# Kerollmops/oxidized-mtbl

Measured on AMD Instinct MI355X. Metric: KV records/s + GiB/s of block bytes decoded, device-resident, higher is better.
Workload: dtype u8; 1 GPU; cfg2: 4 KiB blocks, 16 B keys / 64 B values, restart_interval=16, compression=none, device-resident decode; blocks_per_gpu=100000, block_bytes_per_gpu=401800126, records_per_gpu=5100000, key_bytes_per_gpu=81600000, parallelism=block-sharded x1, no collective

## Files before the change

oxidized-mtbl_amd/csrc/decode.hip:

```cpp
#include <hip/hip_runtime.h>
#include <stdint.h>

#include <stdlib.h>

#include <algorithm>

#include "bounds.h"
#include "devinfo.h"
#include "crc_dev.h"
#include "mtblx.h"

#if (defined(MTBLX_ABL_NOKEY) || defined(MTBLX_ABL_NOVAL) || defined(MTBLX_ABL_NOVSTORE) || \
     defined(MTBLX_ABL_CRC) || defined(MTBLX_SPILL)) && !defined(MTBLX_DIAG)
#error "ablation / spill knobs are diagnostic: build them through a Makefile diagnostic target (-DMTBLX_DIAG)"
#endif

namespace mtblx {

constexpr int kWave = 64;
constexpr uint64_t kU32Max = 0xFFFFFFFFull;
constexpr uint32_t kNotStaged = 0xFFFFFFFFu;
constexpr uint32_t kOutOfBounds = 0xFFFFFFFEu;

__device__ __forceinline__ uint32_t byte_of(const uint4& w, uint32_t t) {
// ... 214 lines not shown
  static constexpr int MAXINT = MAXINT_;
  static constexpr int MAXBLK = MAXBLK_;
  static constexpr bool VALPOS = false;
};

struct Rec {
  uint32_t pos_sh;
  uint32_t ns_vl;
  uint32_t ks;
  uint32_t vs_blk;
};

template <class C>
struct alignas(16) TileLds {
  uint8_t stage[C::TB];
  Rec rec[C::MAXREC];
  uint32_t boff[C::MAXBLK];
  uint32_t blen[C::MAXBLK];
  uint32_t bR[C::MAXBLK];
  uint32_t bn[C::MAXBLK];
  uint32_t bint0[C::MAXBLK + 1];
  uint32_t bok[C::MAXBLK];
  uint32_t bwr[C::MAXBLK];
  int32_t bst[C::MAXBLK];
  uint32_t bcnt[C::MAXBLK], bkb[C::MAXBLK], bvb[C::MAXBLK];
  uint32_t brb[C::MAXBLK], bkbb[C::MAXBLK], bvbb[C::MAXBLK];
  uint32_t brf[C::MAXBLK];
  uint32_t icnt[C::MAXINT + 1], ikb[C::MAXINT + 1], ivb[C::MAXINT + 1];
  uint8_t iblk[C::MAXINT];
  uint64_t tpre[3];
  uint64_t tinc[3];
  uint32_t ttot[3];
  uint32_t nfastrec;
  uint32_t contig;
  uint32_t wsum[4][3];
  uint64_t lbsum[4][3];
};

struct TileArgs {
  const uint8_t* data;
  uint64_t data_len;
  const uint64_t* blk_off;
  const uint32_t* blk_len;
  uint32_t nblk;
  uint32_t bpt;
  uint32_t slot;
  uint32_t ntiles;
  uint32_t* nrec;
  uint64_t* rec_base;
  uint64_t* key_base;
  uint64_t* val_base;
  int32_t* status;
  uint32_t* key_end;
  uint32_t* val_end;
  uint64_t rec_cap;
  uint8_t* keys;
  uint64_t keys_cap;
  uint8_t* vals;
  uint64_t vals_cap;
  uint64_t* totals;
  uint64_t* lbw;
  struct WsHdr* hdr;
  uint64_t* dbg;
  int write;
  uint32_t* crc;
  uint8_t* crc_bad;
  int crc_framed;
  uint32_t wscap;
  uint32_t par;
  uint32_t hw_other;
  unsigned long long inject;
  uint32_t flags_direct;
  uint64_t wait_ticks;
  uint64_t dbg_delay0;
  uint32_t* val_pos;
};

struct WsHdr {
  uint32_t epoch;
  uint32_t done;
  uint32_t hw[2];
  unsigned long long flags;
  unsigned long long tflags[2];
};

__device__ __forceinline__ void tile_span(const TileArgs& a, uint32_t t, uint32_t& b0, uint32_t& nb) {
  b0 = t * a.bpt;
  nb = min(a.bpt, a.nblk - b0);
}

constexpr int kTileWords = 4;
__device__ __forceinline__ uint64_t* lb_slot(const TileArgs& a, uint64_t t) { return a.lbw + kTileWords * t + a.par; }
__device__ __forceinline__ uint64_t* lbx_slot(const TileArgs& a, uint64_t t) { return a.lbw + kTileWords * t + 2; }
__device__ __forceinline__ uint64_t* lbx2_slot(const TileArgs& a, uint64_t t) { return a.lbw + kTileWords * t + 3; }

__device__ __forceinline__ bool fits_at(uint64_t base, uint64_t n, uint64_t cap) { return base <= cap && n <= cap - base; }

__device__ __forceinline__ void ws_begin(TileArgs& a) {
  const uint32_t ep = __hip_atomic_load(&a.hdr->epoch, __ATOMIC_RELAXED, __HIP_MEMORY_SCOPE_AGENT);
  a.par = ep & 1u;
  a.hw_other = __hip_atomic_load(&a.hdr->hw[a.par ^ 1u], __ATOMIC_RELAXED, __HIP_MEMORY_SCOPE_AGENT);
  if (a.hw_other > a.wscap) a.hw_other = a.wscap;
  const uint32_t n = blockDim.x, tid = threadIdx.x;
  for (uint64_t t = (uint64_t)blockIdx.x * n + tid; t < a.hw_other; t += (uint64_t)gridDim.x * n)
    a.lbw[kTileWords * t + (a.par ^ 1u)] = 0;
  if (blockIdx.x == 0 && tid == 0)
    __hip_atomic_store(&a.hdr->tflags[a.par ^ 1u], 0ull, __ATOMIC_RELAXED, __HIP_MEMORY_SCOPE_AGENT);
}

__device__ __forceinline__ void ws_debug_delay(const TileArgs& a) {
  if (blockIdx.x == 0 && a.dbg_delay0) {
    const uint64_t t0 = __builtin_amdgcn_s_memrealtime();
    while (__builtin_amdgcn_s_memrealtime() - t0 < a.dbg_delay0) __builtin_amdgcn_s_sleep(127);
  }
}

__device__ __forceinline__ void ws_flag(const TileArgs& a, unsigned long long bit) {
  atomicOr(a.flags_direct ? reinterpret_cast<unsigned long long*>(a.totals + 3) : &a.hdr->flags, bit);
}

__device__ __forceinline__ void ws_timeout(const TileArgs& a) {
  if (a.flags_direct) {
    __hip_atomic_fetch_or(&a.hdr->tflags[a.par], 2ull, __ATOMIC_RELAXED, __HIP_MEMORY_SCOPE_AGENT);
    asm volatile("s_waitcnt vmcnt(0)" ::: "memory");
  }
  ws_flag(a, 2ull);
}

constexpr uint64_t kWaitTicks = 20ull * 100000000ull;
struct WaitBound {
  uint64_t t0 = 0;
  uint32_t n = 0;
  __device__ __forceinline__ bool expired(uint64_t ticks) {
    if ((++n & 63u) != 0u) return false;
    const uint64_t t = __builtin_amdgcn_s_memrealtime();
    if (t0 == 0) t0 = t;
    return t - t0 > ticks;
  }
};

__device__ __forceinline__ void ws_end(const TileArgs& a) {
  __syncthreads();
  if (threadIdx.x == 0) {
    const uint32_t old = __hip_atomic_fetch_add(&a.hdr->done, 1u, __ATOMIC_RELAXED, __HIP_MEMORY_SCOPE_AGENT);
    if (old == gridDim.x - 1) {
      const unsigned long long f = __hip_atomic_exchange(&a.hdr->flags, 0ull, __ATOMIC_RELAXED, __HIP_MEMORY_SCOPE_AGENT);
      a.totals[3] = f | a.inject;
      __hip_atomic_fetch_max(&a.hdr->hw[a.par], a.ntiles, __ATOMIC_RELAXED, __HIP_MEMORY_SCOPE_AGENT);
      __hip_atomic_exchange(&a.hdr->done, 0u, __ATOMIC_RELAXED, __HIP_MEMORY_SCOPE_AGENT);
      __hip_atomic_fetch_add(&a.hdr->epoch, 1u, __ATOMIC_RELAXED, __HIP_MEMORY_SCOPE_AGENT);
    }
  }
}


__device__ __forceinline__ void pipe_zero_flags(const TileArgs& a) {
  unsigned long long* tot = reinterpret_cast<unsigned long long*>(a.totals + 3);
  __hip_atomic_store(tot, 0ull, __ATOMIC_RELAXED, __HIP_MEMORY_SCOPE_AGENT);
  asm volatile("s_waitcnt vmcnt(0)" ::: "memory");
  const unsigned long long early = __hip_atomic_load(&a.hdr->tflags[a.par], __ATOMIC_RELAXED, __HIP_MEMORY_SCOPE_AGENT);
  if (early) __hip_atomic_fetch_or(tot, early, __ATOMIC_RELAXED, __HIP_MEMORY_SCOPE_AGENT);
  asm volatile("s_waitcnt vmcnt(0)" ::: "memory");
}

__device__ __forceinline__ void pipe_close(const TileArgs& a) {
  if (a.inject) __hip_atomic_fetch_or(a.totals + 3, a.inject, __ATOMIC_RELAXED, __HIP_MEMORY_SCOPE_AGENT);
  __hip_atomic_fetch_max(&a.hdr->hw[a.par], a.ntiles, __ATOMIC_RELAXED, __HIP_MEMORY_SCOPE_AGENT);
  __hip_atomic_fetch_add(&a.hdr->epoch, 1u, __ATOMIC_RELAXED, __HIP_MEMORY_SCOPE_AGENT);
}

__device__ __forceinline__ void tile_range(const TileArgs& a, uint32_t t, uint32_t tb, uint64_t& r0, uint64_t& r1) {
  uint32_t b0, nb;
  tile_span(a, t, b0, nb);
  MTBLX_CHK(a.blk_off + b0, 8 * nb);
  MTBLX_CHK(a.blk_len + b0, 4 * nb);
  const uint64_t s = a.blk_off[b0];
  const uint64_t e = a.blk_off[b0 + nb - 1] + a.blk_len[b0 + nb - 1];
  const uint64_t base = reinterpret_cast<uintptr_t>(a.data);
  r0 = ((base + s) & ~15ull) - base;
  if (base + s < 16 || ((base + s) & ~15ull) < base) r0 = 0;
  r1 = (e > s && e - r0 + 48 <= tb) ? e : 0;
  for (uint32_t j = 1; r1 && j + 1 < nb; ++j)
    if (a.blk_off[b0 + j] < s || a.blk_off[b0 + j] + a.blk_len[b0 + j] > e) r1 = 0;
}

__device__ __forceinline__ uint4 load_chunk(const TileArgs& a, uint64_t off) {
  if (off + 16 <= a.data_len) {
    MTBLX_CHK(a.data + off, 16);
    return *reinterpret_cast<const uint4*>(a.data + off);
  }
  uint32_t t[4] = {0, 0, 0, 0};
  for (int i = 0; i < 16; ++i)
    if (off + i < a.data_len) MTBLX_CHK(a.data + off + i, 1), t[i >> 2] |= (uint32_t)a.data[off + i] << (8 * (i & 3));
  return make_uint4(t[0], t[1], t[2], t[3]);
}

__device__ __forceinline__ uint32_t stage_slot(const TileArgs& a, uint8_t* slot, uint64_t off, uint32_t L, int lane) {
  const uint64_t base = reinterpret_cast<uintptr_t>(a.data);
  const uint64_t a0 = ((base + off) & ~15ull) - base;
  const uint32_t delta = (uint32_t)(off - a0);
  const uint32_t nch = (delta + L + 15u) >> 4;
  for (uint32_t c = lane; c < nch; c += kWave) *reinterpret_cast<uint4*>(slot + 16 * c) = load_chunk(a, a0 + 16ull * c);
  return delta;
}

template <bool WRITE>
__device__ __forceinline__ bool walk_interval(const uint8_t* stage, Rec* recs, uint32_t bo, uint32_t L, uint32_t R, uint32_t s,
                                              uint32_t e, uint32_t& cnt, uint32_t& kb, uint32_t& vb, uint32_t slot0,
                                              uint32_t kbase, uint32_t vbase, uint32_t blk, uint32_t rlo,
                                              uint32_t rhi) {
  cnt = kb = vb = 0;
  if (!(s < e && e <= R)) return false;
  uint32_t p = s, prevlen = 0;
  const uint32_t* st32 = reinterpret_cast<const uint32_t*>(stage);
  while (p < e) {
    const uint32_t ad = bo + p;
    uint32_t hw = (MTBLX_LCHK(st32 + (ad >> 2), 8), __builtin_amdgcn_alignbit(st32[(ad >> 2) + 1], st32[ad >> 2], (ad & 3u) * 8u));
    uint32_t sh = hw & 0xffu, ns = (hw >> 8) & 0xffu, vl = (hw >> 16) & 0xffu, h = 3;
    if (__builtin_expect((hw & 0x808080u) != 0u, 0)) {
      if (R - p < 3u) return false;
      uint4 W = lds_win16(stage, ad);
      uint32_t l0 = dec32(W, 0, L - p, sh);
      if (l0 == 0) return false;
      uint32_t l1 = dec32(W, l0, L - p - l0, ns);
      if (l1 == 0) return false;
      uint32_t l2 = dec32(W, l0 + l1, L - p - l0 - l1, vl);
      if (l2 == 0) return false;
      h = l0 + l1 + l2;
      if (p + h > R) return false;
      if ((sh | ns | vl) > 0xFFFFu) return false;
    }
    if (R - p < h + ns + vl) return false;
    if (sh > prevlen) return false;
    const uint32_t klen = sh + ns;
    if (WRITE) {
      const uint32_t r = slot0 + cnt;
      if (r >= rlo && r < rhi) {
// ... 419 lines not shown
              --sidx;
              const uint32_t x = S.rec[sidx].pos_sh;
              shs = x >> 16;
              ps = x & 0xFFFFu;
            }
            const uint32_t seg = m < jend ? m : jend;
            const uint32_t src = bo + ps + (jj - shs);
            uint4 w4 = lds_win16(S.stage, src - (jj - j0));
            merge_bytes(outw, w4, (int)(jj - j0), (int)(seg - j0));
            jj = seg;
          }
          store_bytes(kd + j0, outw, jend - j0);
        }
#endif
      }
      __syncthreads();
      if (fb >= nint) break;
      plan_chunk(fb);
      walk2();
      __syncthreads();
    }
    STAMP(6);

    if (tid < (int)nb && !S.bok[tid] && S.bwr[tid]) {
      const uint32_t j = tid, bo = S.boff[j], L = S.blen[j];
      const uint8_t* d = (bo != kNotStaged) ? (S.stage + bo) : (a.data + a.blk_off[b0 + j]);
      if constexpr (C::VALPOS)
        generic_block<true, true>(d, L, a.keys + pk + S.bkbb[j], nullptr, a.key_end + pr + S.brb[j],
                                  a.val_end + pr + S.brb[j], a.val_pos + pr + S.brb[j]);
      else
        generic_block<true>(d, L, a.keys + pk + S.bkbb[j], a.vals + pv + S.bvbb[j], a.key_end + pr + S.brb[j],
                            a.val_end + pr + S.brb[j]);
    }
    __syncthreads();
  }
  ws_end(a);
#ifdef MTBLX_STAMPS
  if (tid == 0 && a.dbg) {
    for (int k = 0; k < 8; ++k) atomicAdd(reinterpret_cast<unsigned long long*>(a.dbg + k), (unsigned long long)tacc[k]);
    atomicAdd(reinterpret_cast<unsigned long long*>(a.dbg + 8), (unsigned long long)ntl);
  }
#endif
}

struct Stamps {
#ifdef MTBLX_STAMPS
  uint64_t acc[15] = {0, 0, 0, 0, 0, 0, 0, 0, 0, 0, 0, 0, 0, 0, 0};
  uint64_t prev = 0;
  __device__ __forceinline__ void init() { prev = __builtin_amdgcn_s_memtime(); }
  __device__ __forceinline__ void hit(int k) {
    const uint64_t t = __builtin_amdgcn_s_memtime();
    acc[k] += t - prev;
    prev = t;
  }
#else
  __device__ __forceinline__ void init() {}
  __device__ __forceinline__ void hit(int) {}
#endif
};

#ifdef MTBLX_STAMPS
__device__ uint64_t g_tl[1024][16];
#define TL(k) do { if (threadIdx.x == 0 && blockIdx.x < 1024) g_tl[blockIdx.x][k] = __builtin_amdgcn_s_memrealtime(); } while (0)
#define TLW(k) do { if ((threadIdx.x & 63) == 0 && blockIdx.x < 1024) g_tl[blockIdx.x][k] = __builtin_amdgcn_s_memrealtime(); } while (0)
#else
#define TL(k) do { } while (0)
#define TLW(k) do { } while (0)
#endif

constexpr int kPipeThreads = 1024;
constexpr int kPipeLoadWave = 2;
constexpr int kP2Spi = 16;
constexpr uint32_t kLargeDmaSplit = 24;

template <int TB_, int NBUF_, int MAXBLK_, int MAXINT_, bool VERIFY_ = false, int LOADW_ = 2>
struct PipeCfg {
  static constexpr int TB = TB_, NBUF = NBUF_, MAXBLK = MAXBLK_, MAXINT = MAXINT_;
  static constexpr int SLOTS = MAXINT * kP2Spi;
  static constexpr bool VERIFY = VERIFY_;
  static constexpr int LOADW = LOADW_;
  static constexpr int COPY0 = kPipeLoadWave + LOADW;
  static constexpr int NCOPY = kPipeThreads / kWave - COPY0;
  static constexpr int ROWS = NCOPY * (kWave / 16);
  static constexpr bool VALPOS = false;
};
#ifndef MTBLX_SMALL_TB
#define MTBLX_SMALL_TB 49664
#endif
using PipeSmall = PipeCfg<MTBLX_SMALL_TB, 3, 16, 56>;
#ifndef MTBLX_LARGE_LOADW
#define MTBLX_LARGE_LOADW 2
#endif
using PipeLarge = PipeCfg<65664, 2, 2, 64, false, MTBLX_LARGE_LOADW>;
using PipeSmallV = PipeCfg<49152, 3, 16, 56, true>;
using PipeLargeV = PipeCfg<65664, 2, 2, 64, true>;
struct PipeSmallP : PipeSmall { static constexpr bool VALPOS = true; };
struct PipeLargeP : PipeLarge { static constexpr bool VALPOS = true; };

template <class P>
struct alignas(16) PipeBuf {
  uint8_t stage[P::TB];
  uint16_t pos[P::SLOTS];
  uint32_t boff[P::MAXBLK], blen[P::MAXBLK];
  uint32_t bok[P::MAXBLK], bwr[P::MAXBLK];
  int32_t bst[P::MAXBLK];
  uint32_t bcnt[P::MAXBLK], bkb[P::MAXBLK], bvb[P::MAXBLK];
  uint32_t brb[P::MAXBLK], bkbb[P::MAXBLK], bvbb[P::MAXBLK];
  uint32_t icnt[P::MAXINT + 1], ikb[P::MAXINT + 1], ivb[P::MAXINT + 1];
  uint8_t iraw[P::MAXINT];
  uint8_t iblk[P::MAXINT];
  uint64_t tpre[3];
  uint32_t ttot[3];
  uint32_t nb, b0, nint;
};

template <class P>
struct alignas(16) PipeLds {
  PipeBuf<P> buf[P::NBUF];
  uint32_t ready;
  uint32_t pub;
  uint32_t cdone;
  uint32_t staged;
  uint8_t cmk[kPipeThreads / kWave][kWave];
  uint32_t crcT[P::VERIFY ? 4 : 1][P::VERIFY ? 256 : 1];
  uint32_t cacc[2][P::VERIFY ? P::MAXBLK : 1];
  uint32_t cst[2][P::VERIFY ? P::MAXBLK : 1];
  uint32_t cfr[2][P::VERIFY ? P::MAXBLK : 1];
  uint32_t shK[P::VERIFY ? 64 : 1];
  uint32_t shX[P::VERIFY ? 32 : 1];
  uint32_t crcdone;
};

__device__ __forceinline__ void raw_barrier() {
  asm volatile("s_waitcnt lgkmcnt(0)\n\ts_barrier" ::: "memory");
}

template <int D>
__device__ __forceinline__ uint32_t row_shr_keep(uint32_t x) {
  return (uint32_t)__builtin_amdgcn_update_dpp((int)x, (int)x, 0x110 + D, 0xf, 0xf, false);
}
template <int D>
__device__ __forceinline__ uint32_t row_shr_zero(uint32_t x) {
  return (uint32_t)__builtin_amdgcn_update_dpp(0, (int)x, 0x110 + D, 0xf, 0xf, false);
}

__device__ __forceinline__ uint32_t row_excl_scan(uint32_t x) {
  uint32_t y = x;
  y += row_shr_zero<1>(y);
  y += row_shr_zero<2>(y);
  y += row_shr_zero<4>(y);
  y += row_shr_zero<8>(y);
  return y - x;
}

__device__ __forceinline__ uint32_t keep_mask(int t, int i) {
  int lo = t - 4 * i;
  lo = lo < 0 ? 0 : lo;
  return lo >= 4 ? 0u : (0xFFFFFFFFu << (8 * lo));
}

template <int D>
__device__ __forceinline__ void key_scan_step(uint32_t& m, uint4& W, uint32_t q0) {
  const uint32_t mL = row_shr_keep<D>(m);
  uint4 L;
  L.x = row_shr_keep<D>(W.x);
  L.y = row_shr_keep<D>(W.y);
// ... 113 lines not shown
    kb += klen;
    vb += vl;
    prevlen = klen;
    p += h + ns + vl;
  }
  return p == e && (prevlen <= 0xFFFFu);
}

template <class P>
__device__ __forceinline__ void pipe_dma(PipeBuf<P>& B, const TileArgs& a, uint32_t t, uint64_t off_l, uint32_t len_l,
                                         int lane, uint32_t part, uint32_t mlo = 0, uint32_t mhi = 0xFFFFFFFFu) {
  typedef __attribute__((address_space(3))) void lds_void;
  typedef __attribute__((address_space(1))) const void g_void;
  uint32_t b0, nb;
  tile_span(a, t, b0, nb);
  const uint64_t base = reinterpret_cast<uintptr_t>(a.data);
  const uint64_t s = ((uint64_t)(uint32_t)__builtin_amdgcn_readlane((int)(off_l >> 32), 0) << 32) |
                     (uint32_t)__builtin_amdgcn_readlane((int)(uint32_t)off_l, 0);
  const uint64_t end_l = off_l + len_l;
  const uint64_t e = ((uint64_t)(uint32_t)__builtin_amdgcn_readlane((int)(end_l >> 32), (int)nb - 1) << 32) |
                     (uint32_t)__builtin_amdgcn_readlane((int)(uint32_t)end_l, (int)nb - 1);
  uint64_t r0 = ((base + s) & ~15ull) - base;
  if (base + s < 16 || ((base + s) & ~15ull) < base) r0 = 0;
  const bool inside = off_l >= s && end_l <= e;
  const bool contig = e > s && e - r0 + 48 <= (uint64_t)P::TB && __ballot(!inside) == 0ull;
  if (contig) {
    const uint32_t nch = (uint32_t)((e - r0 + 15) >> 4);
    const bool al = ((base + r0) & 15ull) == 0;
    const uint64_t room = a.data_len > r0 ? (a.data_len - r0) / 16u : 0u;
    const uint32_t nfull = al ? (uint32_t)min<uint64_t>(nch, room) : 0u;
    const uint32_t mfull = min(nfull / kWave, mhi);
    uint32_t m = part + ((mlo + P::LOADW - 1 - part) / P::LOADW) * P::LOADW;
    if (mlo <= part) m = part;
    const uint8_t* gp = a.data + r0 + 16ull * ((uint64_t)m * kWave + (uint32_t)lane);
    for (; m < mfull; m += P::LOADW, gp += 16 * kWave * P::LOADW)
      MTBLX_CHK(gp, 16), MTBLX_LCHK(B.stage + 16 + 1024 * m, 1024), __builtin_amdgcn_global_load_lds((g_void*)gp, (lds_void*)(B.stage + 16 + 1024 * m), 16, 0, MTBLX_DMA_AUX);
    for (; m * kWave < nch && m < mhi; m += P::LOADW) {
      const uint32_t c = m * kWave + lane;
      const uint64_t go = r0 + 16ull * c;
      if (c < nfull)
        MTBLX_CHK(a.data + go, 16), MTBLX_LCHK(B.stage + 16 + 1024 * m, 1024), __builtin_amdgcn_global_load_lds((g_void*)(a.data + go), (lds_void*)(B.stage + 16 + 1024 * m), 16, 0, MTBLX_DMA_AUX);
      else if (c < nch)
        *reinterpret_cast<uint4*>(B.stage + 16 + 16 * c) = load_chunk(a, go);
    }
    if (part == 0 && lane < (int)nb) {
      B.boff[lane] = off_l + len_l > a.data_len ? kOutOfBounds : (uint32_t)(16 + off_l - r0);
      B.blen[lane] = len_l;
    }
  } else if (mlo == 0) {
    for (uint32_t j = 0; j < nb; ++j) {
      const uint64_t off = ((uint64_t)(uint32_t)__builtin_amdgcn_readlane((int)(off_l >> 32), (int)j) << 32) |
                           (uint32_t)__builtin_amdgcn_readlane((int)(uint32_t)off_l, (int)j);
      const uint32_t L = (uint32_t)__builtin_amdgcn_readlane((int)len_l, (int)j);
      const uint32_t so = 16u + j * a.slot;
      uint32_t bo = kNotStaged;
      if (off + L > a.data_len) {
        bo = kOutOfBounds;
      } else if (L + 15u <= a.slot && so + a.slot + 32u <= (uint32_t)P::TB) {
        uint64_t a0 = ((base + off) & ~15ull) - base;
        if (base + off < 16 || ((base + off) & ~15ull) < base) a0 = off;
        const uint32_t delta = (uint32_t)(off - a0);
        const uint32_t nch = (delta + L + 15u) >> 4;
        for (uint32_t m = part; m * kWave < nch; m += P::LOADW) {
          const uint32_t c = m * kWave + lane;
          const uint64_t go = a0 + 16ull * c;
          if (c < nch) {
            if (go + 16 <= a.data_len && ((base + go) & 15ull) == 0)
              MTBLX_CHK(a.data + go, 16), MTBLX_LCHK(B.stage + so + 1024 * m, 1024), __builtin_amdgcn_global_load_lds((g_void*)(a.data + go), (lds_void*)(B.stage + so + 1024 * m), 16, 0,
                                               MTBLX_DMA_AUX);
            else
              *reinterpret_cast<uint4*>(B.stage + so + 16 * c) = load_chunk(a, go);
          }
        }
        bo = so + delta;
      }
      if (part == 0 && lane == 0) { B.boff[j] = bo; B.blen[j] = L; }
    }
  }
  if (part == 0 && lane == 0) { B.nb = nb; B.b0 = b0; }
}

template <class P>
__device__ __forceinline__ void pipe_walk(PipeBuf<P>& B, const TileArgs& a, uint32_t t, int lane, Stamps& ST,
                                          uint32_t& wmode) {
  uint32_t b0, nb;
  tile_span(a, t, b0, nb);
  uint32_t n = 0, R = 0, ok = 0, L = 0, bo = kNotStaged;
  if (lane < (int)nb) {
    L = B.blen[lane];
    bo = B.boff[lane];
    if (bo < kOutOfBounds && L >= 8) {
      n = lds_rd32(B.stage, bo + L - 4);
      if (n != 0 && (uint64_t)(n + 1ull) * 4ull <= L) { R = L - 4u * (n + 1u); ok = 1; }
    }
  }
  uint32_t incl = wave_incl_scan(ok ? n : 0u);
  if (ok && incl > (uint32_t)P::MAXINT) ok = 0;
  n = ok ? n : 0;
  incl = wave_incl_scan(n);
  const uint32_t bint0 = incl - n;
  const uint32_t nint = (uint32_t)__builtin_amdgcn_readlane((int)incl, (int)nb - 1);
  uint32_t j = 0;
  for (uint32_t b = 0; b + 1 < nb; ++b) j += ((uint32_t)__builtin_amdgcn_readlane((int)incl, (int)b) <= (uint32_t)lane);
  const int js = (int)j;
  const uint32_t jbo = (uint32_t)__shfl((int)bo, js, kWave), jR = (uint32_t)__shfl((int)R, js, kWave);
  const uint32_t jn = (uint32_t)__shfl((int)n, js, kWave), jb0 = (uint32_t)__shfl((int)bint0, js, kWave);
  const uint32_t jL = (uint32_t)__shfl((int)L, js, kWave);
  ST.hit(9);
  const bool fl = (uint32_t)lane < nint;
  uint32_t cnt = 0, kb = 0, vb = 0;
  bool wok = false, need2 = false;
  if (fl) {
    const uint32_t i = (uint32_t)lane - jb0;
    const uint32_t s = lds_rd32(B.stage, jbo + jR + 4u * i);
    const uint32_t e = (i + 1 < jn) ? lds_rd32(B.stage, jbo + jR + 4u * (i + 1)) : jR;
    ST.hit(10);
    const uint32_t slot0 = (uint32_t)lane * kP2Spi;
    bool all1 = true;
    constexpr bool kAdaptive = P::NBUF == 2 && !P::VERIFY;
    if (!kAdaptive || wmode == 0u) {
      wok = e <= jR && walk_pos(B.stage, B.pos, jbo, s, e, slot0, cnt, kb, vb);
      if (!wok) {
        wok = e <= jR && walk_pos2(B.stage, B.pos, jbo, s, e, slot0, cnt, kb, vb, all1);
        all1 = false;
      }
    } else {
      wok = e <= jR && walk_pos2(B.stage, B.pos, jbo, s, e, slot0, cnt, kb, vb, all1);
      all1 = all1 || !wok;
    }
    need2 = !all1;
    if (!wok) wok = walk_careful_pos(B.stage, B.pos, jbo, jL, jR, s, e, slot0, cnt, kb, vb);
    B.iraw[lane] = (uint8_t)(cnt < 255u ? cnt : 255u);
    B.iblk[lane] = (uint8_t)j;
  }
  ST.hit(2);
  if constexpr (P::NBUF == 2 && !P::VERIFY) wmode = __ballot(need2) != 0ull ? 1u : 0u;
  const uint64_t failm = __ballot(fl && !wok);
  {
    const uint64_t hi = incl >= 64u ? ~0ull : ((1ull << incl) - 1ull);
    const uint64_t lo = (1ull << bint0) - 1ull;
    if (ok && (failm & hi & ~lo) != 0ull) ok = 0;
  }
  const bool jok = __shfl((int)ok, js, kWave) != 0;
  uint32_t gc = 0, gk = 0, gv = 0;
  int32_t gst = MTBLX_ST_OK;
  if (lane < (int)nb && !ok) {
    if (bo == kNotStaged) MTBLX_CHK(a.blk_off + b0 + lane, 8);
    const uint8_t* d = (bo != kNotStaged) ? (B.stage + bo) : (a.data + a.blk_off[b0 + lane]);
    const GenOut o = bo == kOutOfBounds ? GenOut{0, 0, 0, MTBLX_ST_CORRUPT}
                                        : generic_block<false>(d, L, nullptr, nullptr, nullptr, nullptr);
    gc = o.nrec; gk = (uint32_t)o.kb; gv = (uint32_t)o.vb; gst = o.st;
  }
  const uint32_t gwr = ok || gen_writable(bo, gst);
  const bool reg = fl && jok;
  const uint32_t c = reg ? cnt : 0u, k = reg ? kb : 0u, v = reg ? vb : 0u;
  const uint32_t ic = wave_incl_scan(c), ik = wave_incl_scan(k), iv = wave_incl_scan(v);
  const uint32_t tr = (uint32_t)__builtin_amdgcn_readlane((int)ic, 63) + wave_sum32(gc);
  const uint32_t tk = (uint32_t)__builtin_amdgcn_readlane((int)ik, 63) + wave_sum32(gk);
  const uint32_t tv = (uint32_t)__builtin_amdgcn_readlane((int)iv, 63) + wave_sum32(gv);
  if (lane == 0) {
    if (t == 0) pipe_zero_flags(a);
    lb_publish(a, t, tr, tk, tv);
    B.ttot[0] = tr; B.ttot[1] = tk; B.ttot[2] = tv;
    B.nint = nint;
  }
  if (nb == 1) {
    const uint32_t n0 = (uint32_t)__builtin_amdgcn_readlane((int)incl, 0);
    const uint32_t tc = n0 ? (uint32_t)__builtin_amdgcn_readlane((int)ic, (int)n0 - 1) : 0u;
    const uint32_t tkk = n0 ? (uint32_t)__builtin_amdgcn_readlane((int)ik, (int)n0 - 1) : 0u;
    const uint32_t tvv = n0 ? (uint32_t)__builtin_amdgcn_readlane((int)iv, (int)n0 - 1) : 0u;
    if (lane == 0) {
      B.bok[0] = ok; B.bwr[0] = gwr; B.bst[0] = ok ? MTBLX_ST_OK : gst;
      B.bcnt[0] = ok ? tc : gc; B.bkb[0] = ok ? tkk : gk; B.bvb[0] = ok ? tvv : gv;
      B.brb[0] = 0; B.bkbb[0] = 0; B.bvbb[0] = 0;
    }
    if (fl) {
      B.icnt[lane] = ic - c;
      B.ikb[lane] = ik - k;
      B.ivb[lane] = iv - v;
    }
    return;
  }
  const int ea_l = bint0 ? (int)bint0 - 1 : 0, eb_l = incl ? (int)incl - 1 : 0;
  const uint32_t ea0 = (uint32_t)__shfl((int)ic, ea_l, kWave), eb0 = (uint32_t)__shfl((int)ic, eb_l, kWave);
  const uint32_t ka0 = (uint32_t)__shfl((int)ik, ea_l, kWave), kb0 = (uint32_t)__shfl((int)ik, eb_l, kWave);
  const uint32_t va0 = (uint32_t)__shfl((int)iv, ea_l, kWave), vb0 = (uint32_t)__shfl((int)iv, eb_l, kWave);
  uint32_t bc = 0, bk = 0, bv = 0;
  if (lane < (int)nb) {
    if (ok) {
      bc = (incl ? eb0 : 0u) - (bint0 ? ea0 : 0u);
      bk = (incl ? kb0 : 0u) - (bint0 ? ka0 : 0u);
      bv = (incl ? vb0 : 0u) - (bint0 ? va0 : 0u);
    } else {
      bc = gc; bk = gk; bv = gv;
    }
  }
  const uint32_t jc = wave_incl_scan(bc), jk = wave_incl_scan(bk), jv = wave_incl_scan(bv);
  const uint32_t brb = jc - bc, bkbb = jk - bk, bvbb = jv - bv;
  if (lane < (int)nb) {
    B.bok[lane] = ok; B.bwr[lane] = gwr; B.bst[lane] = ok ? MTBLX_ST_OK : gst;
    B.bcnt[lane] = bc; B.bkb[lane] = bk; B.bvb[lane] = bv;
    B.brb[lane] = brb; B.bkbb[lane] = bkbb; B.bvbb[lane] = bvbb;
  }
  const uint32_t jea = (uint32_t)__shfl((int)(bint0 ? ea0 : 0u), js, kWave);
  const uint32_t jka = (uint32_t)__shfl((int)(bint0 ? ka0 : 0u), js, kWave);
  const uint32_t jva = (uint32_t)__shfl((int)(bint0 ? va0 : 0u), js, kWave);
  const uint32_t jrb = (uint32_t)__shfl((int)brb, js, kWave), jkb = (uint32_t)__shfl((int)bkbb, js, kWave),
                 jvb = (uint32_t)__shfl((int)bvbb, js, kWave);
  if (fl) {
    B.icnt[lane] = jrb + (ic - c) - jea;
    B.ikb[lane] = jkb + (ik - k) - jka;
    B.ivb[lane] = jvb + (iv - v) - jva;
  }
}

__device__ __forceinline__ void pipe_lookback_issue(const TileArgs& a, uint32_t t, uint32_t G,
                                                    uint64_t lbv[kMaxLookbackLoads], int lane) {
  const int64_t lo = (t >= G) ? (int64_t)t - G + 1 : 0;
#pragma unroll
  for (int m = 0; m < kMaxLookbackLoads; ++m) {
    const int64_t i = (int64_t)t - 1 - lane - (int64_t)m * kWave;
    lbv[m] = (i >= lo) ? __hip_atomic_load(lb_slot(a, i), __ATOMIC_RELAXED, __HIP_MEMORY_SCOPE_AGENT) : kReady;
  }
}

__device__ __forceinline__ void pipe_lookback_poll(const TileArgs& a, uint32_t t, uint32_t G,
                                                   uint64_t lbv[kMaxLookbackLoads], int lane, const uint32_t* cdone,
                                                   uint32_t want) {
  const int64_t lo = (t >= G) ? (int64_t)t - G + 1 : 0;
  for (uint32_t spin = 0; spin < (1u << 22); ++spin) {
    bool pend = false;
#pragma unroll
    for (int m = 0; m < kMaxLookbackLoads; ++m) {
      const int64_t i = (int64_t)t - 1 - lane - (int64_t)m * kWave;
      pend |= (i >= lo) && !(lbv[m] & kReady);
    }
    if (__ballot(pend) == 0ull) return;
    if (__hip_atomic_load(cdone, __ATOMIC_RELAXED, __HIP_MEMORY_SCOPE_WORKGROUP) >= want) return;
    __builtin_amdgcn_s_sleep(2);
#pragma unroll
    for (int m = 0; m < kMaxLookbackLoads; ++m) {
      const int64_t i = (int64_t)t - 1 - lane - (int64_t)m * kWave;
      if (i >= lo && !(lbv[m] & kReady)) lbv[m] = __hip_atomic_load(lb_slot(a, i), __ATOMIC_RELAXED, __HIP_MEMORY_SCOPE_AGENT);
    }
  }
}

template <class P>
__device__ __forceinline__ void pipe_lookback(PipeBuf<P>& B, const TileArgs& a, uint32_t t, uint32_t G, uint64_t tinc[3],
                                              uint64_t lbv[kMaxLookbackLoads], int lane, uint32_t* ready,
                                              uint32_t rv) {
  const uint32_t nb = B.nb, b0 = B.b0;
  const int64_t lo = (t >= G) ? (int64_t)t - G + 1 : 0;
  uint64_t sr = 0, sk = 0, sv = 0;
  bool timeout = false;
#pragma unroll
  for (int m = 0; m < kMaxLookbackLoads; ++m) {
    const int64_t i = (int64_t)t - 1 - lane - (int64_t)m * kWave;
    uint64_t w = lbv[m];
    WaitBound wb;
    while (!(w & kReady)) {
      __builtin_amdgcn_s_sleep(2);
      w = __hip_atomic_load(lb_slot(a, i), __ATOMIC_RELAXED, __HIP_MEMORY_SCOPE_AGENT);
      if (wb.expired(a.wait_ticks)) { timeout = true; w = kReady; }
    }
    if (i < lo) continue;
    lb_take(a, (uint64_t)i, w, sr, sk, sv);
  }
  if (timeout) ws_timeout(a);
  sr = lb_wave_sum(sr);
  sv = lb_wave_sum(sv);
  sk = lb_wave_sum(sk);
  const uint64_t pr = tinc[0] + sr, pk = tinc[1] + sk, pv = tinc[2] + sv;
  tinc[0] = pr + B.ttot[0];
  tinc[1] = pk + B.ttot[1];
  tinc[2] = pv + B.ttot[2];
  if (lane == 0) {
    B.tpre[0] = pr; B.tpre[1] = pk; B.tpre[2] = pv;
    if (t == a.ntiles - 1) MTBLX_CHK(a.totals, 24);
    if (t == a.ntiles - 1) { a.totals[0] = tinc[0]; a.totals[1] = tinc[1]; a.totals[2] = tinc[2]; }
  }
  const bool fits = !a.write || (fits_at(pr, B.ttot[0], a.rec_cap) && fits_at(pk, B.ttot[1], a.keys_cap) &&
                                 fits_at(pv, B.ttot[2], a.vals_cap));
  if (fits) {
    __builtin_amdgcn_fence(__ATOMIC_RELEASE, "workgroup");
    if (lane == 0) __hip_atomic_store(ready, rv, __ATOMIC_RELEASE, __HIP_MEMORY_SCOPE_WORKGROUP);
  }
  if (lane < (int)nb) {
    const uint32_t j = lane, b = b0 + j;
    const uint64_t rb = pr + B.brb[j], kb = pk + B.bkbb[j], vb = pv + B.bvbb[j];
    MTBLX_CHK(a.nrec + b, 4);
    MTBLX_CHK(a.rec_base + b, 8);
    MTBLX_CHK(a.key_base + b, 8);
    MTBLX_CHK(a.val_base + b, 8);
    MTBLX_CHK(a.status + b, 4);
    a.nrec[b] = B.bcnt[j];
    a.rec_base[b] = rb;
    a.key_base[b] = kb;
    a.val_base[b] = vb;
    int32_t st = B.bst[j];
    if (a.write && !(fits_at(rb, B.bcnt[j], a.rec_cap) && fits_at(kb, B.bkb[j], a.keys_cap) &&
                     fits_at(vb, B.bvb[j], a.vals_cap))) {
      st = MTBLX_ST_OVERFLOW;
      B.bwr[j] = 0;
      ws_flag(a, 1ull);
    }
    a.status[b] = st;
  }
  if (!fits) {
    __builtin_amdgcn_fence(__ATOMIC_RELEASE, "workgroup");
    if (lane == 0) __hip_atomic_store(ready, rv, __ATOMIC_RELEASE, __HIP_MEMORY_SCOPE_WORKGROUP);
  }
}

struct CopyRow {
  uint32_t f, j, k, bo, sh, ns, vl, klen, ks, vs, sp, m0;
  uint4 W0;
  bool fv, live;
};

template <class P>
__device__ __forceinline__ CopyRow copy_prepare(const PipeBuf<P>& B, uint32_t fb, int lane) {
  CopyRow r;
  const uint32_t nint = B.nint;
  r.k = lane & 15;
  r.f = fb + (lane >> 4);
  r.fv = r.f < nint;
  r.j = r.fv ? B.iblk[r.f] : 0u;
  r.live = r.fv && r.k < B.iraw[r.f] && B.bok[r.j];
  r.bo = B.boff[r.j];
  const uint32_t p = r.live ? B.pos[r.f * kP2Spi + r.k] : 0u;
  uint32_t sh = 0, ns = 0, vl = 0, h = 3;
  if (r.live) {
    const uint32_t hw = lds_rd32(B.stage, r.bo + p);
    sh = hw & 0xffu; ns = (hw >> 8) & 0xffu; vl = (hw >> 16) & 0xffu;
    if ((hw & 0x808080u) != 0u) {
      const uint4 W = lds_win16(B.stage, r.bo + p);
      const uint32_t l0 = dec32(W, 0, 16, sh);
      const uint32_t l1 = dec32(W, l0, 16, ns);
      const uint32_t l2 = dec32(W, l0 + l1, 16, vl);
      h = l0 + l1 + l2;
    }
  }
  r.sh = sh; r.ns = ns; r.vl = vl;
  r.klen = sh + ns;
  const uint32_t kx = row_excl_scan(r.klen), vx = row_excl_scan(vl);
  r.ks = (r.fv ? B.ikb[r.f] : 0u) + kx;
  r.vs = (r.fv ? B.ivb[r.f] : 0u) + vx;
  r.sp = r.bo + p + h;
#ifndef MTBLX_ABL_NOKEY
  const bool own = r.live && sh < 16u && r.klen > 0u;
  uint4 W = own ? lds_win16(B.stage, r.sp - sh) : make_uint4(0, 0, 0, 0);
  uint32_t m = sh;
  key_scan_step<1>(m, W, 0);
  key_scan_step<2>(m, W, 0);
  key_scan_step<4>(m, W, 0);
  key_scan_step<8>(m, W, 0);
  r.W0 = W;
  r.m0 = m;
#endif
  return r;
}

__device__ __forceinline__ uint32_t wave_incl_max(uint32_t x) {
  uint32_t y;
  y = (uint32_t)__builtin_amdgcn_update_dpp(0, (int)x, 0x111, 0xf, 0xf, false); x = x > y ? x : y;
  y = (uint32_t)__builtin_amdgcn_update_dpp(0, (int)x, 0x112, 0xf, 0xf, false); x = x > y ? x : y;
  y = (uint32_t)__builtin_amdgcn_update_dpp(0, (int)x, 0x114, 0xf, 0xf, false); x = x > y ? x : y;
  y = (uint32_t)__builtin_amdgcn_update_dpp(0, (int)x, 0x118, 0xf, 0xf, false); x = x > y ? x : y;
  y = (uint32_t)__builtin_amdgcn_update_dpp(0, (int)x, 0x142, 0xa, 0xf, false); x = x > y ? x : y;
  y = (uint32_t)__builtin_amdgcn_update_dpp(0, (int)x, 0x143, 0xc, 0xf, false); x = x > y ? x : y;
  return x;
}

__device__ __forceinline__ void key_tails_dense(uint8_t* kb, const uint8_t* stage, uint8_t* mk, bool tl, uint32_t klen,
                                                uint32_t src, uint32_t dst, int lane) {
  const uint32_t nc = tl ? (klen - 1u) >> 4 : 0u;
  const uint32_t ci = wave_incl_scan(nc);
  const uint32_t cx = ci - nc;
  const uint32_t C = (uint32_t)__builtin_amdgcn_readlane((int)ci, 63);
  const uint32_t tail = klen - 16u;
  for (uint32_t c0 = 0; c0 < C; c0 += kWave) {
    const uint32_t seed = (uint32_t)__builtin_popcountll(__ballot(ci <= c0));
    mk[lane] = 0;
    if (nc != 0u && cx > c0 && cx < c0 + kWave) mk[cx - c0] = (uint8_t)lane;
    wave_sync();
    uint32_t own = mk[lane];
    own = wave_incl_max(own > seed ? own : seed);
    wave_sync();
    const int o = (int)own;
    const uint32_t ocx = (uint32_t)__shfl((int)cx, o, kWave), osrc = (uint32_t)__shfl((int)src, o, kWave);
    const uint32_t odst = (uint32_t)__shfl((int)dst, o, kWave), otl = (uint32_t)__shfl((int)tail, o, kWave);
    const uint32_t c = c0 + (uint32_t)lane;
    if (c < C) {
      const uint32_t q = 16u * (c - ocx), n = otl - q;
// ... 205 lines not shown
    const uint32_t b = b0 + lane;
    if (a.crc) MTBLX_CHK(a.crc + b, 4);
    if (a.crc_bad) MTBLX_CHK(a.crc_bad + b, 1);
    if (a.crc) a.crc[b] = crc;
    if (a.crc_bad) {
      uint8_t bad = 0;
      if (o == kOutOfBounds) bad = 1;
      else if (a.crc_framed && S.cfr[par][lane]) bad = S.cst[par][lane] != crc;
      a.crc_bad[b] = bad;
    }
  }
}

template <class P>
__device__ __forceinline__ void pipe_crc_copy(const PipeBuf<P>& B, const TileArgs& a, PipeLds<P>& S, uint32_t cw,
                                              int lane, uint32_t par) {
  if constexpr ((MTBLX_ABL_CRC & 4) != 0) return;
  constexpr uint32_t NC = (uint32_t)P::NCOPY;
  const uint32_t nb = B.nb;
  uint32_t stored = 0, framed = 0;
  if (cw == 0 && lane < (int)nb && a.crc_framed && (MTBLX_ABL_CRC & 2) == 0) {
    MTBLX_CHK(a.blk_off + B.b0 + lane, 8);
    const uint64_t off = a.blk_off[B.b0 + lane];
    if (off >= 4 && off <= a.data_len) {
      const uint8_t* d = a.data + off;
      MTBLX_CHK(d - 4, 4);
      stored = (uint32_t)d[-4] | ((uint32_t)d[-3] << 8) | ((uint32_t)d[-2] << 16) | ((uint32_t)d[-1] << 24);
      framed = 1;
    }
  }
  const uint32_t* st32 = reinterpret_cast<const uint32_t*>(B.stage);
  const uint32_t g = nb >= NC ? 1u : NC / nb;
  const uint32_t jstep = nb >= NC ? NC : nb;
  if constexpr ((MTBLX_ABL_CRC & 1) == 0)
  for (uint32_t j = nb >= NC ? cw : cw / g; j < nb; j += jstep) {
    const uint32_t s = nb >= NC ? 0u : cw % g;
    const uint32_t L = B.blen[j], bo = B.boff[j];
    if (bo >= kOutOfBounds || L < 4u) continue;
    const uint32_t nwin = (L + kCrcWinB - 1) / kCrcWinB, nr = (nwin + 63u) / 64u;
    uint32_t acc = 0;
    for (uint32_t r = s; r < nr; r += g) {
      const uint32_t k = (uint32_t)lane + 64u * r;
      uint32_t c = 0;
      if (k < nwin) {
        const int32_t p0 = (int32_t)L - (int32_t)(kCrcWinB * (k + 1u));
        c = lds_window_raw(S, st32, (int32_t)bo + p0, p0);
      }
      acc ^= r ? mtblx_crc::dmultmodp(S.shX[r], c) : c;
    }
    acc = mtblx_crc::dmultmodp(S.shK[lane], acc);
#pragma unroll
    for (int o = 32; o >= 1; o >>= 1) acc ^= (uint32_t)__shfl_xor((int)acc, o, kWave);
    if (lane == 0) __hip_atomic_fetch_xor(&S.cacc[par][j], acc, __ATOMIC_RELAXED, __HIP_MEMORY_SCOPE_WORKGROUP);
  }
  if (cw == 0 && lane < (int)nb) {
    S.cst[par][lane] = stored;
    S.cfr[par][lane] = framed;
  }
  uint32_t old = 0;
  if (lane == 0) old = __hip_atomic_fetch_add(&S.crcdone, 1u, __ATOMIC_ACQ_REL, __HIP_MEMORY_SCOPE_WORKGROUP);
  old = (uint32_t)__builtin_amdgcn_readfirstlane((int)old);
  if (old % NC != NC - 1) return;
  __builtin_amdgcn_fence(__ATOMIC_ACQUIRE, "workgroup");
  pipe_crc_final(B, a, S, lane, par);
}

#ifdef MTBLX_SPILL
constexpr int kSpillPad = MTBLX_SPILL;
#else
constexpr int kSpillPad = 0;
#endif
template <class P>
__global__ void __launch_bounds__(kPipeThreads, 1) k_decode_pipe(TileArgs a) {
  uint32_t spill_pad[kSpillPad > 0 ? kSpillPad : 1];
  if constexpr (kSpillPad > 0) {
#pragma unroll
    for (int i = 0; i < kSpillPad; ++i) spill_pad[i] = a.blk_len[((uint32_t)threadIdx.x + 7u * i) % a.nblk];
  }
  __shared__ PipeLds<P> S;
  constexpr bool kSerial = P::NBUF == 2 && P::VERIFY;
  constexpr bool kLate = P::NBUF == 2 && !P::VERIFY;
  const int tid = threadIdx.x, lane = tid & 63, wv = tid >> 6;
  const uint32_t g = blockIdx.x, G = gridDim.x;
  const uint32_t nloc = (a.ntiles > g) ? (a.ntiles - g + G - 1) / G : 0;
  Stamps ST;
  ST.init();
  TL(0);
  ws_begin(a);
  if constexpr (!P::VERIFY) ws_debug_delay(a);
  a.flags_direct = 1;
  if (tid == 0) { S.ready = 0; S.pub = 0; S.cdone = 0; S.crcdone = 0; S.staged = 0; }
  if constexpr (P::VERIFY) {
    for (int i = tid; i < 4 * 256; i += kPipeThreads) S.crcT[i >> 8][i & 255] = mtblx_crc::kTab.slice[i >> 8][i & 255];
    for (int i = tid; i < 2 * P::MAXBLK; i += kPipeThreads) S.cacc[i / P::MAXBLK][i % P::MAXBLK] = 0;
    if (tid < 64) S.shK[tid] = mtblx_crc::xpow8((uint64_t)kCrcWinB * (uint32_t)tid);
    else if (tid < 64 + (int)kCrcRounds) S.shX[tid - 64] = mtblx_crc::xpow8((uint64_t)kCrcWinB * 64u * (uint32_t)(tid - 64));
  }

  uint64_t tinc[3] = {0, 0, 0};
  uint64_t lbv[kMaxLookbackLoads];
  uint64_t ioff = 0;
  uint32_t ilen = 0;
  auto load_info = [&](uint32_t kk) {
    if (kk >= nloc) return;
    uint32_t b0, nb;
    tile_span(a, g + kk * G, b0, nb);
    const uint32_t j = (uint32_t)lane < nb ? (uint32_t)lane : nb - 1;
    MTBLX_CHK(a.blk_off + b0 + j, 8);
    MTBLX_CHK(a.blk_len + b0 + j, 4);
    ioff = a.blk_off[b0 + j];
    ilen = a.blk_len[b0 + j];
  };
  const bool loader = wv >= kPipeLoadWave && wv < kPipeLoadWave + P::LOADW;
  const uint32_t part = (uint32_t)(wv - kPipeLoadWave);
  if (loader) {
    load_info(0);
    if constexpr (!kLate) {
      if (nloc > 0) pipe_dma(S.buf[0], a, g, ioff, ilen, lane, part);
      load_info(1);
    }
    asm volatile("s_waitcnt vmcnt(0)" ::: "memory");
  } else if (wv == 1) {
    if (!kSerial && nloc > 0) pipe_lookback_issue(a, g, G, lbv, lane);
  }
  __syncthreads();
  TL(1);
  if (wv == 0) __builtin_amdgcn_s_setprio(2);
  uint64_t ntl = 0;
  uint32_t wmode = 0;

  if constexpr (kSerial) {
    for (uint32_t it = 0; it < nloc; ++it) {
      PipeBuf<P>& C = S.buf[it & 1u];
      const uint32_t tc = g + it * G;
      if (wv == 0) {
        pipe_walk(C, a, tc, lane, ST, wmode);
        __builtin_amdgcn_fence(__ATOMIC_RELEASE, "workgroup");
        if (lane == 0) __hip_atomic_store(&S.pub, it + 1, __ATOMIC_RELEASE, __HIP_MEMORY_SCOPE_WORKGROUP);
        ST.hit(3);
      } else if (loader) {
        if (it + 1 < nloc) {
          PipeBuf<P>& N = S.buf[(it + 1) & 1u];
          const bool late = it >= 1 && 3ull * N.ttot[1] <= (uint64_t)N.ttot[2];
          pipe_dma(N, a, tc + G, ioff, ilen, lane, part, 0, late ? kLargeDmaSplit : 0xFFFFFFFFu);
          if (late) {
            wait_flag(a, &S.pub, it + 1);
            pipe_dma(N, a, tc + G, ioff, ilen, lane, part, kLargeDmaSplit);
          }
          load_info(it + 2);
        }
        ST.hit(4);
        asm volatile("s_waitcnt vmcnt(0)" ::: "memory");
        ST.hit(6);
      } else if (wv == 1) {
        wait_flag(a, &S.pub, it + 1);
        pipe_lookback_issue(a, tc, G, lbv, lane);
        pipe_lookback(C, a, tc, G, tinc, lbv, lane, &S.ready, it + 1);
        ST.hit(1);
      } else {
        wait_flag(a, &S.pub, it + 1);
        pipe_copy(C, a, wv - P::COPY0, lane, &S.ready, it + 1, ST, S.cmk[wv]);
        pipe_crc_copy(C, a, S, (uint32_t)(wv - P::COPY0), lane, it & 1u);
        ST.hit(7);
      }
      raw_barrier();
      if (wv == 0) { ST.hit(8); ++ntl; }
      else if (wv == P::COPY0) ST.hit(5);
      else if (loader) ST.hit(12);
      else ST.hit(1);
    }
  } else if constexpr (kLate) {
    for (int it = -1; it < (int)nloc; ++it) {
      const uint32_t k1 = (uint32_t)(it + 1);
      if (wv == 0) {
        if (k1 < nloc) {
          wait_flag(a, &S.staged, (k1 + 1) * (uint32_t)P::LOADW);
          ST.hit(8);
          pipe_walk(S.buf[k1 & 1u], a, g + k1 * G, lane, ST, wmode);
          if (lane == 0) __hip_atomic_store(&S.pub, k1 + 1, __ATOMIC_RELAXED, __HIP_MEMORY_SCOPE_WORKGROUP);
        }
        ST.hit(3);
      } else if (loader) {
        if (k1 < nloc) {
          pipe_dma(S.buf[k1 & 1u], a, g + k1 * G, ioff, ilen, lane, part);
          load_info(k1 + 1);
          asm volatile("s_waitcnt vmcnt(0)" ::: "memory");
          __builtin_amdgcn_fence(__ATOMIC_RELEASE, "workgroup");
          if (lane == 0) __hip_atomic_fetch_add(&S.staged, 1u, __ATOMIC_RELEASE, __HIP_MEMORY_SCOPE_WORKGROUP);
        }
        ST.hit(4);
        ST.hit(6);
      } else if (it >= 0) {
        PipeBuf<P>& C = S.buf[(uint32_t)it & 1u];
        const uint32_t tc = g + (uint32_t)it * G;
        if (wv == 1) {
          pipe_lookback(C, a, tc, G, tinc, lbv, lane, &S.ready, (uint32_t)it + 1);
          if (it + 1 == (int)nloc) TLW(8);
          else if (it + 2 == (int)nloc) TLW(11);
          ST.hit(1);
          if (k1 < nloc) {
            WaitBound wb;
            while (__hip_atomic_load(&S.pub, __ATOMIC_RELAXED, __HIP_MEMORY_SCOPE_WORKGROUP) < k1 + 1) {
              __builtin_amdgcn_s_sleep(1);
              if (wb.expired(handoff_ticks(a))) { ws_timeout(a); break; }
            }
            pipe_lookback_issue(a, tc + G, G, lbv, lane);
            pipe_lookback_poll(a, tc + G, G, lbv, lane, &S.cdone, (uint32_t)(it + 1) * P::NCOPY);
          }
          ST.hit(1);
        } else {
          pipe_copy(C, a, wv - P::COPY0, lane, &S.ready, (uint32_t)it + 1, ST, S.cmk[wv]);
          if (wv == P::COPY0 && it + 1 == (int)nloc) TLW(9);
          if (wv == P::COPY0 + P::NCOPY - 1 && it + 1 == (int)nloc) TLW(10);
          if (lane == 0) __hip_atomic_fetch_add(&S.cdone, 1u, __ATOMIC_RELAXED, __HIP_MEMORY_SCOPE_WORKGROUP);
          ST.hit(7);
        }
      }
      raw_barrier();
      if (it == -1) TL(2);
      else if (it == 0) TL(3);
      else if (it + 2 == (int)nloc) TL(7);
      if (wv == 0) { ST.hit(8); ++ntl; }
      else if (wv >= P::COPY0) ST.hit(5);
      else if (loader) ST.hit(12);
      else ST.hit(11);
    }
  } else
  for (int it = -1; it < (int)nloc; ++it) {
    const uint32_t k1 = (uint32_t)(it + 1), k2 = (uint32_t)(it + 2);
    if (wv == 0) {
      if (k1 < nloc) {
        pipe_walk(S.buf[k1 % P::NBUF], a, g + k1 * G, lane, ST, wmode);
        if (lane == 0) __hip_atomic_store(&S.pub, k1 + 1, __ATOMIC_RELAXED, __HIP_MEMORY_SCOPE_WORKGROUP);
      }
      ST.hit(3);
    } else if (loader) {
      if (k2 < nloc) {
        pipe_dma(S.buf[k2 % P::NBUF], a, g + k2 * G, ioff, ilen, lane, part);
        load_info(k2 + 1);
      }
      ST.hit(4);
      asm volatile("s_waitcnt vmcnt(0)" ::: "memory");
      ST.hit(6);
    } else if (it >= 0) {
      PipeBuf<P>& C = S.buf[(uint32_t)it % P::NBUF];
      const uint32_t tc = g + (uint32_t)it * G;
      if (wv == 1) {
        pipe_lookback(C, a, tc, G, tinc, lbv, lane, &S.ready, (uint32_t)it + 1);
        if (it + 1 == (int)nloc) TLW(8);
        else if (it + 2 == (int)nloc) TLW(11);
        ST.hit(1);
        if (k1 < nloc) {
          WaitBound wb;
          while (__hip_atomic_load(&S.pub, __ATOMIC_RELAXED, __HIP_MEMORY_SCOPE_WORKGROUP) < k1 + 1) {
            __builtin_amdgcn_s_sleep(1);
            if (wb.expired(handoff_ticks(a))) { ws_timeout(a); break; }
          }
          pipe_lookback_issue(a, tc + G, G, lbv, lane);
          pipe_lookback_poll(a, tc + G, G, lbv, lane, &S.cdone, (uint32_t)(it + 1) * P::NCOPY);
        }
        ST.hit(1);
      } else {
        pipe_copy(C, a, wv - P::COPY0, lane, &S.ready, (uint32_t)it + 1, ST, S.cmk[wv]);
        if (wv == P::COPY0 && it + 1 == (int)nloc) TLW(9);
        if (wv == P::COPY0 + P::NCOPY - 1 && it + 1 == (int)nloc) TLW(10);
        if (lane == 0) __hip_atomic_fetch_add(&S.cdone, 1u, __ATOMIC_RELAXED, __HIP_MEMORY_SCOPE_WORKGROUP);
        if constexpr (P::VERIFY) pipe_crc_copy(C, a, S, (uint32_t)(wv - P::COPY0), lane, (uint32_t)it & 1u);
        ST.hit(7);
      }
    }
    raw_barrier();
    if (it == -1) TL(2);
    else if (it == 0) TL(3);
    else if (it + 2 == (int)nloc) TL(7);
    if (wv == 0) { ST.hit(8); ++ntl; }
    else if (wv >= P::COPY0) ST.hit(5);
    else if (loader) ST.hit(12);
    else ST.hit(11);
  }
  TL(4);
  asm volatile("s_waitcnt vmcnt(0)" ::: "memory");
  if (wv >= P::COPY0) TLW(12 + (wv & 1));
  TLW(14 + (wv == 1));
  if (g == (a.ntiles - 1) % G && tid == 0) pipe_close(a);
  if constexpr (kSpillPad > 0) {
#pragma unroll
    for (int i = 0; i < kSpillPad; ++i) asm volatile("" ::"v"(spill_pad[i]));
  }
  TL(5);
#ifdef MTBLX_STAMPS
  if (tid == 0 && blockIdx.x < 1024) g_tl[blockIdx.x][6] = nloc;
#endif
#ifdef MTBLX_STAMPS
  __shared__ unsigned long long cmin, cmax;
  if (tid == 0) { cmin = ~0ull; cmax = 0; }
  __syncthreads();
  if (lane == 0 && wv >= P::COPY0) {
    atomicMin(&cmin, (unsigned long long)ST.acc[5]);
    atomicMax(&cmax, (unsigned long long)ST.acc[14]);
  }
  __syncthreads();
  if (tid == 0 && a.dbg) {
    atomicAdd(reinterpret_cast<unsigned long long*>(a.dbg + 13), cmin);
    atomicAdd(reinterpret_cast<unsigned long long*>(a.dbg + 14), cmax);
  }
  if (lane == 0 && a.dbg && (wv <= kPipeLoadWave || wv == P::COPY0)) {
    for (int k = 0; k < 13; ++k) {
      const bool mine = (wv == 0) ? (k == 2 || k == 3 || k == 8 || k == 9 || k == 10) : (wv == 1) ? (k == 1 || k == 11) : loader ? (k == 4 || k == 6 || k == 12) : (k == 0 || k == 5 || k == 7);
      if (mine) atomicAdd(reinterpret_cast<unsigned long long*>(a.dbg + k), (unsigned long long)ST.acc[k]);
    }
    if (wv == 0) atomicAdd(reinterpret_cast<unsigned long long*>(a.dbg + 15), (unsigned long long)ntl);
  }
#else
  (void)ntl;
#endif
// ... 152 lines not shown
```

Baseline: 2505 GiB/s.

## Adapt blocks-per-tile from prior call's observed restart-interval count hint

The walk wave now records the largest per-block restart count it sees into a device-side header field. The last tile hands this value over for the next launch. On the next call, ws_begin reads the hint and shrinks blocks-per-tile and the tile count so that a tile's restart intervals fit the MAXINT slot capacity. This is meant to avoid overflow or fallback paths when blocks carry more restarts than the static tiling assumes. It relies on state carried across calls, adds atomics and a vmcnt wait near the final tiles, and changes the tile count on later calls.

```diff
diff --git a/oxidized-mtbl_amd/csrc/decode.hip b/oxidized-mtbl_amd/csrc/decode.hip
--- a/oxidized-mtbl_amd/csrc/decode.hip
+++ b/oxidized-mtbl_amd/csrc/decode.hip
@@ -320,6 +320,8 @@
   uint32_t hw[2];
   unsigned long long flags;
   unsigned long long tflags[2];
+  uint32_t ipb_cur;
+  uint32_t ipb_next;
 };
 
 __device__ __forceinline__ void tile_span(const TileArgs& a, uint32_t t, uint32_t& b0, uint32_t& nb) {
@@ -334,8 +336,17 @@
 
 __device__ __forceinline__ bool fits_at(uint64_t base, uint64_t n, uint64_t cap) { return base <= cap && n <= cap - base; }
 
-__device__ __forceinline__ void ws_begin(TileArgs& a) {
+__device__ __forceinline__ void ws_begin(TileArgs& a, uint32_t hint_cap = 0) {
   const uint32_t ep = __hip_atomic_load(&a.hdr->epoch, __ATOMIC_RELAXED, __HIP_MEMORY_SCOPE_AGENT);
+  if (hint_cap) {
+    const uint32_t ipb = (uint32_t)__builtin_amdgcn_readfirstlane(
+        (int)__hip_atomic_load(&a.hdr->ipb_cur, __ATOMIC_RELAXED, __HIP_MEMORY_SCOPE_AGENT));
+    if ((uint64_t)ipb * a.bpt > hint_cap) {
+      const uint32_t fit = ipb >= hint_cap ? 1u : hint_cap / ipb;
+      a.bpt = (uint32_t)__builtin_amdgcn_readfirstlane((int)fit);
+      a.ntiles = (uint32_t)__builtin_amdgcn_readfirstlane((int)((a.nblk - 1) / fit + 1));
+    }
+  }
   a.par = ep & 1u;
   a.hw_other = __hip_atomic_load(&a.hdr->hw[a.par ^ 1u], __ATOMIC_RELAXED, __HIP_MEMORY_SCOPE_AGENT);
   if (a.hw_other > a.wscap) a.hw_other = a.wscap;
@@ -391,6 +402,11 @@
   }
 }
 
+
+__device__ __forceinline__ void pipe_hint_handover(const TileArgs& a) {
+  const uint32_t ipb = __hip_atomic_exchange(&a.hdr->ipb_next, 0u, __ATOMIC_RELAXED, __HIP_MEMORY_SCOPE_AGENT);
+  __hip_atomic_store(&a.hdr->ipb_cur, ipb, __ATOMIC_RELAXED, __HIP_MEMORY_SCOPE_AGENT);
+}
 
 __device__ __forceinline__ void pipe_zero_flags(const TileArgs& a) {
   unsigned long long* tot = reinterpret_cast<unsigned long long*>(a.totals + 3);
@@ -976,6 +992,7 @@
   static constexpr int COPY0 = kPipeLoadWave + LOADW;
   static constexpr int NCOPY = kPipeThreads / kWave - COPY0;
   static constexpr int ROWS = NCOPY * (kWave / 16);
+  static constexpr int HINTCAP = MAXINT;
   static constexpr bool VALPOS = false;
 };
 #ifndef MTBLX_SMALL_TB
@@ -1255,7 +1272,7 @@
 
 template <class P>
 __device__ __forceinline__ void pipe_walk(PipeBuf<P>& B, const TileArgs& a, uint32_t t, int lane, Stamps& ST,
-                                          uint32_t& wmode) {
+                                          uint32_t& wmode, uint32_t& ipbseen) {
   uint32_t b0, nb;
   tile_span(a, t, b0, nb);
   uint32_t n = 0, R = 0, ok = 0, L = 0, bo = kNotStaged;
@@ -1265,6 +1282,17 @@
     if (bo < kOutOfBounds && L >= 8) {
       n = lds_rd32(B.stage, bo + L - 4);
       if (n != 0 && (uint64_t)(n + 1ull) * 4ull <= L) { R = L - 4u * (n + 1u); ok = 1; }
+    }
+  }
+  if constexpr (!(P::NBUF == 2 && P::VERIFY)) {
+    const uint32_t hn = (ok && n <= (uint32_t)P::HINTCAP) ? n : 0u;
+    uint64_t more = __ballot(hn > ipbseen);
+    if (more != 0ull) {
+      do {
+        ipbseen = (uint32_t)__builtin_amdgcn_readlane((int)hn, (int)__builtin_ctzll(more));
+        more = __ballot(hn > ipbseen);
+      } while (more != 0ull);
+      if (lane == 0) __hip_atomic_fetch_max(&a.hdr->ipb_next, ipbseen, __ATOMIC_RELAXED, __HIP_MEMORY_SCOPE_AGENT);
     }
   }
   uint32_t incl = wave_incl_scan(ok ? n : 0u);
@@ -1331,6 +1359,7 @@
   const uint32_t tr = (uint32_t)__builtin_amdgcn_readlane((int)ic, 63) + wave_sum32(gc);
   const uint32_t tk = (uint32_t)__builtin_amdgcn_readlane((int)ik, 63) + wave_sum32(gk);
   const uint32_t tv = (uint32_t)__builtin_amdgcn_readlane((int)iv, 63) + wave_sum32(gv);
+  if (t + gridDim.x >= a.ntiles) asm volatile("s_waitcnt vmcnt(0)" ::: "memory");
   if (lane == 0) {
     if (t == 0) pipe_zero_flags(a);
     lb_publish(a, t, tr, tk, tv);
@@ -1484,6 +1513,7 @@
     __builtin_amdgcn_fence(__ATOMIC_RELEASE, "workgroup");
     if (lane == 0) __hip_atomic_store(ready, rv, __ATOMIC_RELEASE, __HIP_MEMORY_SCOPE_WORKGROUP);
   }
+  if (t == a.ntiles - 1 && lane == 0) pipe_hint_handover(a);
 }
 
 struct CopyRow {
@@ -1855,11 +1885,11 @@
   constexpr bool kLate = P::NBUF == 2 && !P::VERIFY;
   const int tid = threadIdx.x, lane = tid & 63, wv = tid >> 6;
   const uint32_t g = blockIdx.x, G = gridDim.x;
-  const uint32_t nloc = (a.ntiles > g) ? (a.ntiles - g + G - 1) / G : 0;
   Stamps ST;
   ST.init();
   TL(0);
-  ws_begin(a);
+  ws_begin(a, P::HINTCAP);
+  const uint32_t nloc = (a.ntiles > g) ? (a.ntiles - g + G - 1) / G : 0;
   if constexpr (!P::VERIFY) ws_debug_delay(a);
   a.flags_direct = 1;
   if (tid == 0) { S.ready = 0; S.pub = 0; S.cdone = 0; S.crcdone = 0; S.staged = 0; }
@@ -1901,13 +1931,14 @@
   if (wv == 0) __builtin_amdgcn_s_setprio(2);
   uint64_t ntl = 0;
   uint32_t wmode = 0;
+  uint32_t ipbseen = 0;
 
   if constexpr (kSerial) {
     for (uint32_t it = 0; it < nloc; ++it) {
       PipeBuf<P>& C = S.buf[it & 1u];
       const uint32_t tc = g + it * G;
       if (wv == 0) {
-        pipe_walk(C, a, tc, lane, ST, wmode);
+        pipe_walk(C, a, tc, lane, ST, wmode, ipbseen);
         __builtin_amdgcn_fence(__ATOMIC_RELEASE, "workgroup");
         if (lane == 0) __hip_atomic_store(&S.pub, it + 1, __ATOMIC_RELEASE, __HIP_MEMORY_SCOPE_WORKGROUP);
         ST.hit(3);
@@ -1949,7 +1980,7 @@
         if (k1 < nloc) {
           wait_flag(a, &S.staged, (k1 + 1) * (uint32_t)P::LOADW);
           ST.hit(8);
-          pipe_walk(S.buf[k1 & 1u], a, g + k1 * G, lane, ST, wmode);
+          pipe_walk(S.buf[k1 & 1u], a, g + k1 * G, lane, ST, wmode, ipbseen);
           if (lane == 0) __hip_atomic_store(&S.pub, k1 + 1, __ATOMIC_RELAXED, __HIP_MEMORY_SCOPE_WORKGROUP);
         }
         ST.hit(3);
@@ -2003,7 +2034,7 @@
     const uint32_t k1 = (uint32_t)(it + 1), k2 = (uint32_t)(it + 2);
     if (wv == 0) {
       if (k1 < nloc) {
-        pipe_walk(S.buf[k1 % P::NBUF], a, g + k1 * G, lane, ST, wmode);
+        pipe_walk(S.buf[k1 % P::NBUF], a, g + k1 * G, lane, ST, wmode, ipbseen);
         if (lane == 0) __hip_atomic_store(&S.pub, k1 + 1, __ATOMIC_RELAXED, __HIP_MEMORY_SCOPE_WORKGROUP);
       }
       ST.hit(3);
```

Result: slower. 2448 GiB/s (-2.3%).
